# empymod/emg3d

Hardware: AMD Instinct MI355X
Metric: Mcells/s per multigrid cycle (higher is better)
Workload: dtype c128

## Files before the change

emg3d_amd/csrc/mg.hpp:

```cpp
#pragma once
#include <algorithm>
#include <cmath>
#include <cstdlib>
#include <cstring>
#include <map>
#include <memory>
#include <mutex>
#include <chrono>
#include <vector>

#include "common.hpp"
#include "smooth.hpp"
#include "stencil.hpp"
#include "smooth_qpl.hpp"
#include "smooth_qc.hpp"
#include "smooth_thm.hpp"
#include "smooth_tha.hpp"
#include "sweep_launch.hpp"
#include "sweep_plan.hpp"

template <class T>
struct Level {
    i64 nC[3];
    i64 nE, nCells;
// ... 869 lines not shown
        a.fac = L.fac[dir];
        a.fcomp = L.fac_kind[dir] == 4;
        if (L.fac_kind[dir] == 3) {
            a.mid = L.fac_mid[dir];
            const i64 nQ_ = L.nC[a.Q];
            const i64 nmax_ = a.nA[0] * ((nQ_ - 0) / 2);
            a.mode = 3;
            if (nmax_ > 0)
                MG_LAUNCH(k_line_factor_m<T>, dim3((unsigned)((nmax_ + EMG_LINE_BLOCK - 1) / EMG_LINE_BLOCK), 4),
                                   dim3(EMG_LINE_BLOCK), 0, stream, a);
            check_launch();
            return;
        }
        a.mid = L.fac_mid[dir];
        const i64 nQ = L.nC[a.Q];
        const i64 nB[2] = {(nQ - 0) / 2, (nQ - 1) / 2};
        a.mode = 3; a.cP = a.cQ = 0; a.cntA = a.cntB = 0;
        const i64 nmax = a.nA[0] * nB[0];
#ifdef EMG3D_LAB
        if (LAB_ENV("EMG3D_FACTOR_PER_COLOUR", 0)) {
            for (int c = 0; c < 4; ++c) {
                a.mode = 0; a.cP = c & 1; a.cQ = c >> 1; a.cntA = a.nA[a.cP]; a.cntB = nB[a.cQ];
                const i64 n = a.cntA * a.cntB;
                if (n > 0)
                    MG_LAUNCH(k_line_factor<T>, dim3((unsigned)((n + EMG_LINE_BLOCK - 1) / EMG_LINE_BLOCK)),
                                       dim3(EMG_LINE_BLOCK), 0, stream, a);
            }
            check_launch();
            return;
        }
#endif
        if (nmax > 0)
            MG_LAUNCH(k_line_factor<T>, dim3((unsigned)((nmax + EMG_LINE_BLOCK - 1) / EMG_LINE_BLOCK), 4),
                               dim3(EMG_LINE_BLOCK), 0, stream, a);
        check_launch();
    }

    unsigned xcd_grid(i64 nb) const { return (unsigned)(xcd_map ? ((nb + 7) / 8) * 8 : nb); }
    unsigned rp_grid(i64 nt) const { return xcd_grid((nt + EMG_RP_BLOCK - 1) / EMG_RP_BLOCK); }
    void ensure_qdesc(Level<T>& L, int dir) {
        const SweepPlan& P = plan(L, dir);
        if (!P.qdesc || L.qd[dir][0] || L.qdn[dir][0] == ~0u) return;
        L.qdn[dir][0] = ~0u;
        if (!L.fac[dir]) return;
        LineArgs<T> a;
        line_args(L, dir, a, true);
        const i64 lpg = 16 / a.seg;
        a.bt = Batch();
        for (int c = 0; c < 4; ++c) {
            a.mode = 0; a.cP = c & 1; a.cQ = c >> 1;
            a.cntA = a.nA[a.cP]; a.cntB = a.nB2[a.cQ];
            a.rs.slot0 = (unsigned)a.base[c];
            const i64 n = a.cntA * a.cntB;
            if (n <= 0) continue;
            const unsigned grid = xcd_grid((n + lpg - 1) / lpg);
            const i64 nthreads = (i64)grid * 64;
            void* tab = try_alloc<char>(nthreads * a.qM * (3 * 16 + 8 * 16));
            if (!tab) return;
            a.qd = tab; a.qdn = (unsigned)nthreads;
            if (!broken) qpl_launch<T>(1, a.qM, false, 1, false, dim3(grid), stream, a);
            L.qd[dir][c] = tab; L.qdn[dir][c] = (unsigned)nthreads;
        }
        check_launch();
    }
    char sweep_name[64] = "";
    char res_name[64] = "";
    int thm_lifo = (int)LAB_ENV("EMG3D_THM_LIFO", 0);
    void thm_attrs() {
#ifdef EMG3D_LAB
        static bool done[64] = {false};
        if (device < 0 || device >= 64 || done[device]) return;
        done[device] = true;
        thm_lifo_attrs<T>();
#endif
    }
    void launch_sweep(const SweepPlan& P, const LineArgs<T>& a, i64 n) {
        if (log_launches) fprintf(stderr, "[sweep] nC %lld %lld %lld L %d lines %lld kernel %s split %d\n", (long long)a.nC[0], (long long)a.nC[1], (long long)a.nC[2], a.L, (long long)n,
                                  P.name, a.split);
        memcpy(sweep_name, P.name, sizeof sweep_name);
        if (broken) return;
        switch (P.family) {
        case SweepFamily::tha: {
            const size_t dyn = P.helpers == 2 ? tha_lds_bytes<T, 2>((int)a.nC[a.L]) : tha_lds_bytes<T, 3>((int)a.nC[a.L]);
            tha_launch<T>(P.helpers, a.zsep != 0, bgrid(xcd_grid((n + THA_LPW - 1) / THA_LPW)), dyn, stream, a);
            break;
        }
        case SweepFamily::thm: {
            const i64 npairs = (n + P.inst_lpw - 1) / P.inst_lpw;
            thm_launch<T>(P.stages, P.inst_lpw, thm_lifo != 0, a.zsep != 0, bgrid(rp_grid(npairs * 128)), stream, a);
            break;
        }
        case SweepFamily::qpl:
        case SweepFamily::qpl_chain: {
            const i64 lpg = (16 * P.NW) / P.seg;
            qpl_launch<T>(P.NW, P.M, false, (P.NW == 1 && a.qd) ? 2 : 0, P.family == SweepFamily::qpl_chain,
                          bgrid(xcd_grid((n + lpg - 1) / lpg)), stream, a);
            break;
        }
        case SweepFamily::qc:
        case SweepFamily::qc_big: {
            LineArgs<T> b = a;
            b.qlpw = P.inst_lpw == 16 ? sweep_balanced_lpw(knobs, n * nsys) : P.inst_lpw;
            qc_launch<T>(P.stages, P.inst_lpw, a.zsep != 0, P.big, bgrid(rp_grid(((n + b.qlpw - 1) / b.qlpw) * 64)), stream, b);
            break;
        }
        case SweepFamily::rp: {
            const unsigned g = rp_grid(((n + P.inst_lpw - 1) / P.inst_lpw) * 64);
            if (P.inst_lpw == 8) hipLaunchKernelGGL((k_line_sweep_rp<T, 8>), bgrid(g), dim3(EMG_RP_BLOCK), 0, stream, a);
            else if (P.inst_lpw == 12) hipLaunchKernelGGL((k_line_sweep_rp<T, 12>), bgrid(g), dim3(EMG_RP_BLOCK), 0, stream, a);
            else hipLaunchKernelGGL((k_line_sweep_rp<T, 4>), bgrid(g), dim3(EMG_RP_BLOCK), 0, stream, a);
            break;
        }
        case SweepFamily::tpl:
            hipLaunchKernelGGL(k_line_sweep<T>, bgrid_y((unsigned)((n + EMG_LINE_BLOCK - 1) / EMG_LINE_BLOCK)), dim3(EMG_LINE_BLOCK), 0, stream, a);
            break;
        }
    }

    void prepare_work(Level<T>& L, int dir) {
        ensure_sflags(L, dir);
        if (home_on(L) || home_lvl(L)) ensure_work(L, 1);
        if (split_on(L)) ensure_work(L, (dir == 0) ? 0 : 1);
        else if (plan(L, dir).xt) ensure_transposed_model(L);
    }
    void to_work(Level<T>& L, int dir) {
        ensure_sflags(L, dir);
        if (split_on(L)) {
            const int w = (dir == 0) ? 0 : 1;
            ensure_work(L, w);
            if (home_lvl(L)) {
                if (w == 0) {
                    if (!L.sW_valid[0]) { convert_field(L, L.sW[0], L.sW[1], 2, true); L.sW_valid[0] = true; }
                    convert_field(L, L.eW[0], L.eW[1], 2, true);
                }
                return;
            }
            if (!L.sW_valid[w]) { convert_field(L, L.sW[w], L.s, w, true); L.sW_valid[w] = true; }
            if (!home_on(L)) convert_field(L, L.eW[w], L.e, w, true);
            else {
                e_to_w1(L);
                if (w == 0) convert_field(L, L.eW[0], L.eW[1], 2, true);
            }
        } else if (plan(L, dir).xt) {
            if (!L.sT_valid) { convert_field(L, L.sT, L.s, -1, true); L.sT_valid = true; }
            convert_field(L, L.eT, L.e, -1, true);
        }
    }
    void from_work(Level<T>& L, int dir) {
        if (home_on(L) || home_lvl(L)) {
            if (dir == 0) convert_field(L, L.eW[1], L.eW[0], 2, false);
        } else if (split_on(L)) convert_field(L, L.e, L.eW[(dir == 0) ? 0 : 1], (dir == 0) ? 0 : 1, false);
        else if (plan(L, dir).xt) convert_field(L, L.e, L.eT, -1, false);
    }
    int work_id(Level<T>& L, int dir) { return plan(L, dir).work_id; }

    int place_tries = getenv("EMG3D_PLACE_TRIES") ? atoi(getenv("EMG3D_PLACE_TRIES")) : 12;
    i64 place_min_bytes = LAB_ENV("EMG3D_PLACE_MIN_MB", 256) << 20;
    int place_reps = (int)LAB_ENV("EMG3D_PLACE_REPS", 1);
    double place_gap = 1.075;
    static const int PLACE_MAX = 16;
    struct PlaceRec { int tries = 0, kept = 0, reused = 0; float ms[PLACE_MAX] = {0}; };
    PlaceRec place_rec[2];
    bool placed[2] = {false, false};
    static bool lr_has(int lr, int dir) {
        return dir == 0 ? (lr == 1 || lr == 5 || lr == 6 || lr == 7) : dir == 1 ? (lr == 2 || lr == 4 || lr == 6 || lr == 7)
                                                                              : (lr == 3 || lr == 4 || lr == 5 || lr == 7);
    }
// ... 419 lines not shown
```

emg3d_amd/csrc/smooth_tha.hpp:

```cpp
#pragma once
#include "smooth_thm.hpp"

struct ThaPair { double a, b; };

constexpr int THA_LPW = 8;
constexpr int THA_MAX_DYN_LDS = 140 * 1024;
constexpr int THA_STATIC_LDS = 18 * 1024;
template <int NH> constexpr int tha_ring_depth() { return 8; }
template <class T, int NH>
inline size_t tha_lds_bytes(int nL) {
    const size_t KS = (size_t)((nL + 1) / 2);
    return ((size_t)2 * tha_ring_depth<NH>() * 5 + (size_t)2 * (KS + 2)) * (5 * THA_LPW) * sizeof(T);
}

template <int NH> constexpr int tha_threads() { return 64 * (2 + 2 * NH); }
template <class T, int NH, bool ZS = false>
__global__ __launch_bounds__(tha_threads<NH>()) void k_line_sweep_tha(LineArgs<T> a) {
    typedef unsigned int u32;
    constexpr int LPW = THA_LPW, D = tha_ring_depth<NH>(), NW = tha_threads<NH>() / 64, L40 = 5 * LPW;
    const int lane = threadIdx.x & 63;
    const int wave = __builtin_amdgcn_readfirstlane(threadIdx.x >> 6);
    const int H = wave & 1;
    const int hj = (wave >> 1) - 1;
    const int q = lane / LPW;
    const int g = lane - q * LPW;
    thm_args_burst(a);
    __shared__ int prod[2][4];
    __shared__ int cons[2];
    __shared__ int mid[2];
    if (threadIdx.x < 8) (&prod[0][0])[threadIdx.x] = 0;
    if (threadIdx.x >= 8 && threadIdx.x < 10) cons[threadIdx.x - 8] = 0;
    if (threadIdx.x >= 10 && threadIdx.x < 12) mid[threadIdx.x - 10] = 0;
    __syncthreads();
#ifdef EMG3D_LAB
    const bool ts_on = (a.tile & 256) && blockIdx.x == 0 && lane == 0 && H == 0;
    long long ts[6] = {0, 0, 0, 0, 0, 0};
    __shared__ long long ts0;
#define THA_TS(i) do { if (ts_on) ts[i] = (long long)__builtin_readcyclecounter(); } while (0)
    if (ts_on && hj < 0) ts0 = (long long)__builtin_readcyclecounter();
#else
#define THA_TS(i) do {} while (0)
#endif
    THA_TS(0);
    EMG_SWEEP_WG(a)
    const u32 gidx = (u32)wg * LPW + g;
    const u32 cA = (u32)a.cntA;
    if (gidx >= cA * (u32)a.cntB) return;
    const u32 bq = gidx / cA, qq = gidx - bq * cA;
    const u32 jP = 1u + (u32)a.cP + 2u * qq, jQ = 1u + (u32)a.cQ + 2u * bq;
    const int n = (int)a.rs.nL;
    const int m = (int)a.mid;
    const int K = H ? n - m - 2 : m;
    const int KS = (n + 1) / 2;
    const u32 slot = a.rs.slot0 + gidx;
    const u32 nLt = (u32)a.nLinesTot;
    const u32 csL = a.rs.csL, csP = a.rs.csP, csQ = a.rs.csQ;
    const double ihP[2] = {a.rs.ihP[jP - 1], a.rs.ihP[jP]};
    const double ihQ[2] = {a.rs.ihQ[jQ - 1], a.rs.ihQ[jQ]};
    const double kP[2] = {0.5 * ihP[0], 0.5 * ihP[1]};
    const double kQ[2] = {0.5 * ihQ[0], 0.5 * ihQ[1]};
    const u32 jPm = jP - 1, jPp = jP + 1, jQm = jQ - 1, jQp = jQ + 1;
    const bool spl = (a.split & 1) != 0;
    const u32 nPc = a.rs.nP, nPn = a.rs.nP + 1u;
    const u32 spsh = spl ? 1u : 0u, sphc = spl ? (nPc + 1u) >> 1 : 0u, sphn = spl ? (nPn + 1u) >> 1 : 0u;
    auto spc = [&](u32 v) -> u32 { return (v >> spsh) + (v & spsh) * sphc; };
    auto spn = [&](u32 v) -> u32 { return (v >> spsh) + (v & spsh) * sphn; };
#define FL_(vL, vP, vQ) (a.rs.off[0] + (vL) * a.rs.st[0][0] + spn(vP) * a.rs.st[0][1] + (vQ) * a.rs.st[0][2])
#define FP_(vL, vP, vQ) (a.rs.off[1] + (vL) * a.rs.st[1][0] + spc(vP) * a.rs.st[1][1] + (vQ) * a.rs.st[1][2])
#define FQ_(vL, vP, vQ) (a.rs.off[2] + (vL) * a.rs.st[2][0] + spn(vP) * a.rs.st[2][1] + (vQ) * a.rs.st[2][2])
    const u32 cP0 = spc(jP - 1) * csP, cP1 = spc(jP) * csP, cq = (jQ - 1) * csQ;

    const bool rowact = q < 5;
    const int rr = rowact ? q : 0;
    const int type = (rr == 0) ? 0 : (rr <= 2 ? 1 : 2);
    const int side = (rr == 0) ? 0 : ((rr - 1) & 1);
    const double sg = side ? -1.0 : 1.0;
    const double tmask = (type == 0) ? 0.0 : 1.0;
    u32 ob[7], os[7];
    u32 fb, sv, suT0;
    double Kc[6];
    double ca = 0.0;
    if (type == 0) {
        ob[0] = FL_(0, jP, jQ);
        ob[1] = FL_(0, jPp, jQ); ob[2] = FL_(0, jPm, jQ); ob[3] = FL_(0, jP, jQp); ob[4] = FL_(0, jP, jQm);
        ob[5] = ob[1]; ob[6] = ob[1];
#pragma unroll
        for (int t = 0; t < 7; ++t) os[t] = a.rs.st[0][0];
        fb = cP0 + cq; sv = csQ; suT0 = cP1 - cP0;
        Kc[0] = kP[1] * ihP[1]; Kc[1] = kP[0] * ihP[0]; Kc[2] = kQ[1] * ihQ[1]; Kc[3] = kQ[0] * ihQ[0];
        Kc[4] = 0.0; Kc[5] = 0.0;
    } else if (type == 1) {
        const u32 pcell = jPm + side, pnode = side ? jPp : jPm;
        ob[0] = FP_(1, pcell, jQ);
        ob[1] = FL_(1, pnode, jQ); ob[2] = FL_(0, pnode, jQ);
        ob[3] = FQ_(1, pnode, jQ); ob[4] = FQ_(1, pnode, jQm);
        ob[5] = FP_(1, pcell, jQp); ob[6] = FP_(1, pcell, jQm);
        os[0] = a.rs.st[1][0]; os[1] = a.rs.st[0][0]; os[2] = a.rs.st[0][0];
        os[3] = a.rs.st[2][0]; os[4] = a.rs.st[2][0]; os[5] = a.rs.st[1][0]; os[6] = a.rs.st[1][0];
        fb = (side ? cP1 : cP0) + cq; sv = csQ; suT0 = 0;
        const double ihA = ihP[side];
        Kc[0] = sg * ihA; Kc[1] = -sg * ihA;
        Kc[2] = sg * kQ[1] * ihA; Kc[3] = -sg * kQ[0] * ihA;
        Kc[4] = kQ[1] * ihQ[1]; Kc[5] = kQ[0] * ihQ[0];
        ca = sg * 0.5 * ihA;
    } else {
        const u32 qcell = jQm + side, qnode = side ? jQp : jQm;
        ob[0] = FQ_(1, jP, qcell);
        ob[1] = FL_(1, jP, qnode); ob[2] = FL_(0, jP, qnode);
// ... 44 lines not shown
    const u32 wst = 15u * nLt * TS;
    u32 eo[6], es[6];
#pragma unroll
    for (int t = 0; t < 6; ++t) { eo[t] = ob[1 + t] * TS; es[t] = os[1 + t] * TS; }
    const u32 so = ob[0] * TS, ss = os[0] * TS;
    const u32 zo0 = fb * 8u, zo1 = (fb + sv) * 8u;
    const u32 zsu = suT0 * 8u, zsL = csL * 8u;

    extern __shared__ __attribute__((aligned(16))) char tha_dyn_lds[];
    const int l40 = rr * LPW + g;
    T* const ring = reinterpret_cast<T*>(tha_dyn_lds) + (size_t)H * (D * 5 * L40) + l40;
    T* const zs = reinterpret_cast<T*>(tha_dyn_lds) + (size_t)2 * (D * 5 * L40) + (size_t)H * ((KS + 2) * L40);
    __shared__ T xy_[NW][64];
    __shared__ ThaPair xc_[NW][64];
    __shared__ T jn[2][6 * LPW];
    T* const xy = xy_[wave];
    ThaPair* const xc = xc_[wave];

    auto own_idx = [&](int ic) -> u32 {
        int v = t0 ? ic : (H ? ic - 1 : ic);
        const int hi = t0 ? n - 1 : n - 2;
        v = v < 0 ? 0 : (v > hi ? hi : v);
        return (u32)v;
    };
    auto fwd_block = [&](int k) -> int { return H ? n - 1 - k : k; };
    auto bwd_block = [&](int k) -> int { return H ? m + 2 + k : m - 1 - k; };
    auto rhs = [&](const TmStep<T>& cur, double& czb, double& cza, double& kLb, double& kLa) -> T {
        kLb = 0.5 * cur.ihl0; kLa = 0.5 * cur.ihl1;
        const double f0 = ZS ? zeta_of(0, cur.zf[0]) : cur.zf[0], f1 = ZS ? zeta_of(1, cur.zf[0]) : cur.zf[1];
        const double f2 = ZS ? zeta_of(2, cur.zf[2]) : cur.zf[2], f3 = ZS ? zeta_of(3, cur.zf[2]) : cur.zf[3];
        const double rs0 = f0 + f1, rs1 = f2 + f3;
        const double cs0 = f0 + f2, cs1 = f1 + f3;
        const double g0 = (t0 ? Kc[0] : Kc[0] * kLa) * rs1;
        const double g1 = (t0 ? Kc[1] : Kc[1] * kLb) * rs0;
        T y = cur.S;
        y += g0 * cur.E[0];
        y += g1 * cur.E[1];
        y += (Kc[2] * cs1) * cur.E[2];
        y += (Kc[3] * cs0) * cur.E[3];
        y += (Kc[4] * cs1) * cur.E[4];
        y += (Kc[5] * cs0) * cur.E[5];
        czb = rs0 * cur.ihl0;
        cza = rs1 * cur.ihl1;
        return y;
    };
    auto load_rhs = [&](u32 ix, TmStep<T>& d) {
        const u32 su = t0 ? zsu : zsL;
        const u32 zb = __umul24(ix, zsL);
        if (ZS) {
            d.zf[0] = *reinterpret_cast<const double*>(wLB + ix * 8u);
            d.zf[2] = *reinterpret_cast<const double*>(wLB + (t0 ? ix : ix + 1u) * 8u);
        } else {
            d.zf[0] = *reinterpret_cast<const double*>(zB + (zb + zo0));
            d.zf[1] = *reinterpret_cast<const double*>(zB + (zb + zo1));
            d.zf[2] = *reinterpret_cast<const double*>(zB + (zb + zo0 + su));
            d.zf[3] = *reinterpret_cast<const double*>(zB + (zb + zo1 + su));
        }
        d.ihl0 = *reinterpret_cast<const double*>(hB + ix * 8u);
        d.ihl1 = *reinterpret_cast<const double*>(hB + (t0 ? ix : ix + 1u) * 8u);
        d.S = nosrc ? Zero<T>::v() : *reinterpret_cast<const T*>(sB + (so + __umul24(ix, ss)));
#pragma unroll
        for (int t = 0; t < 6; ++t) d.E[t] = *reinterpret_cast<const T*>(eB + (eo[t] + __umul24(ix, es[t])));
    };
#ifdef EMG3D_LAB
    long long ts_wait = 0;
#endif
    auto wait_ge = [&](int* p, int v, int& seen) {
        if (seen >= v) return;
#ifdef EMG3D_LAB
        const long long w0 = ts_on ? (long long)__builtin_readcyclecounter() : 0;
#endif
        while ((seen = __hip_atomic_load(p, __ATOMIC_ACQUIRE, __HIP_MEMORY_SCOPE_WORKGROUP)) < v) __builtin_amdgcn_s_sleep(1);
#ifdef EMG3D_LAB
        if (ts_on) ts_wait += (long long)__builtin_readcyclecounter() - w0;
#endif
    };

    if (hj >= 0) {
        if (!rowact) return;
        int cons_seen = 0;
        auto publish = [&](int gs) {
            if (lane == 0) __hip_atomic_store(&prod[H][hj], gs + 1, __ATOMIC_RELEASE, __HIP_MEMORY_SCOPE_WORKGROUP);
        };
        auto load_f = [&](int k_, TmStep<T>& d) {
            const int ic_ = fwd_block(k_ < K ? k_ : K - 1);
            load_rhs(own_idx(ic_), d);
            const u32 wb = __umul24((u32)ic_, wst);
#pragma unroll
            for (int c = 0; c < 5; ++c) d.W[c] = *reinterpret_cast<const T*>(wB + (wb + wo[c]));
        };
        auto produce_f = [&](const TmStep<T>& cur, int k_) {
            double czb, cza, kLb, kLa;
            const T y = rhs(cur, czb, cza, kLb, kLa);
            const double cz = H ? cza : czb;
            const double kk = H ? kLa : kLb;
            ThaPair cc; cc.a = (tmask * kk) * cz; cc.b = cah * cz;
            xy[lane] = y;
            xc[lane] = cc;
            const T Y0 = xy[g], Y1 = xy[g + LPW], Y2 = xy[g + 2 * LPW], Y3 = xy[g + 3 * LPW], Y4 = xy[g + 4 * LPW];
            const ThaPair C1 = xc[g + LPW], C2 = xc[g + 2 * LPW], C3 = xc[g + 3 * LPW], C4 = xc[g + 4 * LPW];
            const T av = ((cur.W[0] * Y0 + cur.W[1] * Y1) + (cur.W[2] * Y2 + cur.W[3] * Y3)) + cur.W[4] * Y4;
            const T G1 = cur.W[1] * C1.a - cur.W[0] * C1.b, G2 = cur.W[2] * C2.a - cur.W[0] * C2.b;
            const T G3 = cur.W[3] * C3.a - cur.W[0] * C3.b, G4 = cur.W[4] * C4.a - cur.W[0] * C4.b;
            wait_ge(&cons[H], k_ - D + 1, cons_seen);
            if (rowact) {
                T* const s_ = ring + (size_t)((u32)k_ % (u32)D) * (5 * L40);
                s_[0] = av; s_[L40] = G1; s_[2 * L40] = G2; s_[3 * L40] = G3; s_[4 * L40] = G4;
            }
            publish(k_);
        };
        THA_TS(1);
        {
            TmStep<T> bA, bB;
            int k = hj;
            if (k < K) load_f(k, bA);
            for (; k < K; k += 2 * NH) {
                if (k + NH < K) load_f(k + NH, bB);
                produce_f(bA, k);
                if (k + NH < K) {
                    if (k + 2 * NH < K) load_f(k + 2 * NH, bA);
                    produce_f(bB, k + NH);
                }
            }
        }
        THA_TS(2);
        struct BwdIn { T W[5]; double p0, p1, ihc; };
        auto load_b = [&](int kb_, BwdIn& d) {
            const int ic_ = bwd_block(kb_);
            const u32 wb = __umul24((u32)ic_, wst);
#pragma unroll
            for (int c = 1; c < 5; ++c) d.W[c] = *reinterpret_cast<const T*>(wB + (wb + wo[c]));
            const int ci = H ? ic_ - 1 : ic_ + 1;
            const u32 zb = __umul24((u32)ci, zsL);
            if (ZS) {
                d.p0 = *reinterpret_cast<const double*>(wLB + (u32)ci * 8u);
            } else {
                d.p0 = *reinterpret_cast<const double*>(zB + (zb + zo0));
                d.p1 = *reinterpret_cast<const double*>(zB + (zb + zo1));
            }
            d.ihc = *reinterpret_cast<const double*>(hB + (u32)ci * 8u);
        };
        auto produce_b = [&](const BwdIn& bc, int kb_) {
            const double cz = (ZS ? zeta_of(0, bc.p0) + zeta_of(1, bc.p0) : bc.p0 + bc.p1) * bc.ihc;
            ThaPair cc; cc.a = cah * cz; cc.b = ((-0.5 * tmask) * bc.ihc) * cz;
            xc[lane] = cc;
            const ThaPair C1 = xc[g + LPW], C2 = xc[g + 2 * LPW], C3 = xc[g + 3 * LPW], C4 = xc[g + 4 * LPW];
            const T h0 = (bc.W[1] * C1.a + bc.W[2] * C2.a) + (bc.W[3] * C3.a + bc.W[4] * C4.a);
            const int gs = K + kb_;
            wait_ge(&cons[H], gs - D + 1, cons_seen);
            if (rowact) {
                T* const s_ = ring + (size_t)((u32)gs % (u32)D) * (5 * L40);
                s_[0] = -h0; s_[L40] = -(bc.W[1] * C1.b); s_[2 * L40] = -(bc.W[2] * C2.b);
                s_[3 * L40] = -(bc.W[3] * C3.b); s_[4 * L40] = -(bc.W[4] * C4.b);
            }
            publish(gs);
        };
        {
            BwdIn bA, bB;
            int k = hj;
            if (k < K) load_b(k, bA);
            for (; k < K; k += 2 * NH) {
                if (k + NH < K) load_b(k + NH, bB);
                produce_b(bA, k);
                if (k + NH < K) {
                    if (k + 2 * NH < K) load_b(k + 2 * NH, bA);
                    produce_b(bB, k + NH);
                }
            }
        }
        THA_TS(3);
#ifdef EMG3D_LAB
        if (ts_on) printf("[tha helper %d] entry %lld setup %lld fwd done %lld bwd done %lld (cycles after the chain wave's entry), waiting for ring space %lld\n",
                          hj, ts[0] - ts0, ts[1] - ts0, ts[2] - ts0, ts[3] - ts0, ts_wait);
#endif
        return;
    }

    const int icm = H ? m + 1 : m;
    TmStep<T> cur;
    load_rhs((u32)(t0 ? icm : m), cur);
    const int ur = H ? 5 : rr;
    T Wm[6];
#pragma unroll
    for (int c = 0; c < 6; ++c) {
        const int r1 = ur > c ? ur : c, c1 = ur > c ? c : ur;
        const int p = r1 * (r1 + 1) / 2 + c1;
        const u32 blk = p < 15 ? (u32)m : (u32)m + 1u;
        const int ent = p < 15 ? p : p - 15;
        Wm[c] = *reinterpret_cast<const T*>(wB + (__umul24(blk, wst) + ((u32)ent * nLt + slot) * TS));
    }
    int prod_seen[NH];
#pragma unroll
    for (int j = 0; j < NH; ++j) prod_seen[j] = 0;
    auto consumed = [&](int gs) {
        asm volatile("" ::: "memory");
        if (lane == 0) __hip_atomic_store(&cons[H], gs + 1, __ATOMIC_RELAXED, __HIP_MEMORY_SCOPE_WORKGROUP);
    };
    THA_TS(1);
    T* const zrow = zs + l40;
    const T* const zcol = zs + g;
    zrow[0] = Zero<T>::v();
    T zprev = Zero<T>::v();
    auto fwd_step = [&](int k_, int j_) {
        wait_ge(&prod[H][j_], k_ + 1, prod_seen[j_]);
        const T* const s_ = ring + (size_t)((u32)k_ % (u32)D) * (5 * L40);
        const T av = s_[0], G1 = s_[L40], G2 = s_[2 * L40], G3 = s_[3 * L40], G4 = s_[4 * L40];
        const T* const zc = zcol + (size_t)k_ * L40;
        const T Z1 = zc[LPW], Z2 = zc[2 * LPW], Z3 = zc[3 * LPW], Z4 = zc[4 * LPW];
        T z = av;
        T z2 = G2 * Z2;
        cmac(z, G1, Z1);
        cmac(z2, G4, Z4);
        cmac(z, G3, Z3);
        z = z + z2;
        zrow[(size_t)(k_ + 1) * L40] = z;
        zprev = z;
        consumed(k_);
    };
    {
        int k = 0;
        for (; k + NH <= K; k += NH) {
#pragma unroll
            for (int j = 0; j < NH; ++j) fwd_step(k + j, j);
        }
#pragma unroll
        for (int j = 0; j < NH; ++j) if (k + j < K) fwd_step(k + j, j);
    }
    THA_TS(2);
#ifdef EMG3D_LAB
    ts[5] = ts_wait;
#endif
    auto pair_sync = [&](int epoch) {
        if (lane == 0) __hip_atomic_store(&mid[H], epoch, __ATOMIC_RELEASE, __HIP_MEMORY_SCOPE_WORKGROUP);
        while (__hip_atomic_load(&mid[1 - H], __ATOMIC_ACQUIRE, __HIP_MEMORY_SCOPE_WORKGROUP) < epoch) __builtin_amdgcn_s_sleep(1);
    };
    pair_sync(1);
    {
        double czb, cza, kLb, kLa;
        T y = rhs(cur, czb, cza, kLb, kLa);
        const T zL = H ? Zero<T>::v() : zprev;
        const int KR = n - m - 2;
        const T zR = (reinterpret_cast<T*>(tha_dyn_lds) + (size_t)2 * (D * 5 * L40) + (size_t)((KS + 2) * L40))[(size_t)KR * L40 + l40];
        if (!H) {
            y += ((tmask * kLb) * czb) * zL;
            y += ((tmask * kLa) * cza) * zR;
            xy[lane] = (ca * czb) * zL;
        } else {
            xy[lane] = (ca * cza) * zR;
        }
        const T su = (xy[g + LPW] + xy[g + 2 * LPW]) + (xy[g + 3 * LPW] + xy[g + 4 * LPW]);
        if (t0) y = H ? y + su : y - su;
        if (rowact) {
            if (!H) jn[0][rr * LPW + g] = y;
            else if (t0) jn[0][5 * LPW + g] = y;
        }
        pair_sync(2);
        T x = Zero<T>::v();
#pragma unroll
        for (int c = 0; c < 6; ++c) x += Wm[c] * jn[0][c * LPW + g];
        if (rowact && (!H || t0)) jn[1][(H ? 5 : rr) * LPW + g] = x;
        pair_sync(3);
        if (rowact && (!H || t0)) {
            if (!H) *reinterpret_cast<T*>(eWr + (so + __umul24((u32)m, ss))) = x;
            else *reinterpret_cast<T*>(eWr + (so + __umul24((u32)(m + 1), ss))) = x;
        }
        zprev = jn[1][(t0 ? (H ? 5 : 0) : rr) * LPW + g];
        zrow[(size_t)(K + 1) * L40] = zprev;
    }
    THA_TS(3);
    u32 xo = so + __umul24(own_idx(bwd_block(0)), ss);
    const u32 dxo = H ? ss : 0u - ss;
    auto bwd_step = [&](int kb_, int j_) {
        const int gs = K + kb_;
        wait_ge(&prod[H][j_], gs + 1, prod_seen[j_]);
        const T* const s_ = ring + (size_t)((u32)gs % (u32)D) * (5 * L40);
        const T H0 = s_[0], H1 = s_[L40], H2 = s_[2 * L40], H3 = s_[3 * L40], H4 = s_[4 * L40];
        const int kz = K - kb_;
        const T zi = zrow[(size_t)kz * L40];
        const T* const xc_in = zcol + (size_t)(kz + 1) * L40;
        const T X0 = xc_in[0], X1 = xc_in[LPW], X2 = xc_in[2 * LPW], X3 = xc_in[3 * LPW], X4 = xc_in[4 * LPW];
        T x = zi;
        T x2 = H1 * X1;
        cmac(x, H0, X0);
        cmac(x2, H3, X3);
        cmac(x, H2, X2);
        cmac(x2, H4, X4);
        x = x + x2;
        zrow[(size_t)kz * L40] = x;
        *reinterpret_cast<T*>(eWr + xo) = x;
        xo += dxo;
        consumed(gs);
    };
    {
        int k = 0;
        for (; k + NH <= K; k += NH) {
#pragma unroll
            for (int j = 0; j < NH; ++j) bwd_step(k + j, j);
        }
#pragma unroll
        for (int j = 0; j < NH; ++j) if (k + j < K) bwd_step(k + j, j);
    }
    THA_TS(4);
#ifdef EMG3D_LAB
    if (ts_on) printf("[tha chain L] K %d: setup %lld forward %lld middle %lld backward %lld (cycles after entry), waiting for helpers %lld (%lld of it in the forward steps)\n", K,
                      ts[1] - ts[0], ts[2] - ts[0], ts[3] - ts[0], ts[4] - ts[0], ts_wait, ts[5]);
#endif
#undef THA_TS
}
```

emg3d_amd/csrc/sweep_launch.hpp:

```cpp
#pragma once
#include "smooth.hpp"
#include "stencil.hpp"

template <class T> void qc_launch(int stages, int lpw, bool zsep, bool big, dim3 grid, hipStream_t st, const LineArgs<T>& a);

template <class T> void thm_launch(int stages, int lpw, bool lifo, bool zsep, dim3 grid, hipStream_t st, const LineArgs<T>& a);
template <class T> void thm_lifo_attrs();

template <class T> void tha_launch(int helpers, bool zsep, dim3 grid, size_t dyn_lds, hipStream_t st, const LineArgs<T>& a);
template <class T> bool tha_attrs(int max_dyn_lds);

template <class T> void qpl_launch(int nw, int m, bool hl, int dm, bool chain, dim3 grid, hipStream_t st, const LineArgs<T>& a);

template <class T> void residual_launch(int mode, int kz, dim3 grid, hipStream_t st, const ResidualArgs<T>& a);
```

emg3d_amd/csrc/sweep_plan.hpp:

```cpp
#pragma once
#include <algorithm>
#include <cstdint>
#include <cstdio>
#include <cstdlib>

typedef int64_t i64;

#ifndef LAB_ENV
#ifdef EMG3D_LAB
inline long long lab_env_(const char* name, long long def) { const char* v = getenv(name); return v ? atoll(v) : def; }
inline int lab_env_ch_(const char* name) { const char* v = getenv(name); return v ? v[0] : 0; }
#define LAB_ENV(name, def) lab_env_(name, (long long)(def))
#define LAB_ENV_CH(name) lab_env_ch_(name)
#else
#define LAB_ENV(name, def) ((long long)(def))
#define LAB_ENV_CH(name) 0
#endif
#endif

constexpr int SWEEP_THA_LPW = 8, SWEEP_THA_RING = 8, SWEEP_THA_MAX_DYN_LDS = 140 * 1024, SWEEP_THA_STATIC_LDS = 18 * 1024;
inline i64 sweep_tha_lds_bytes(i64 nL, int tsize) {
    return (2 * SWEEP_THA_RING * 5 + 2 * ((nL + 1) / 2 + 2)) * (5 * SWEEP_THA_LPW) * (i64)tsize;
}

struct SweepKnobs {
    i64 simds = 1024;
    i64 lds_limit = 160 * 1024;
    bool tha_lds_granted = true;
    int order = 1, nsys = 1;
    int batch_tune = getenv("EMG3D_BATCH_TUNE") ? atoi(getenv("EMG3D_BATCH_TUNE")) : 0;

    int sweep_kernel = LAB_ENV_CH("EMG3D_SWEEP") == 't' ? 1 : 0;
    bool use_xt = LAB_ENV("EMG3D_XT", 1) != 0;
    i64 xt_min_cells = LAB_ENV("EMG3D_XT_MIN", 8192);
    int th_lpw = (int)LAB_ENV("EMG3D_TH_LPW", 0);
    int force_lpw = (int)LAB_ENV("EMG3D_LPW", 0);
    bool use_twist = LAB_ENV("EMG3D_TWIST", 1) != 0;
    i64 twist_max_lines_env = LAB_ENV("EMG3D_TWIST_MAX", 0);
    int tw_stages = (int)LAB_ENV("EMG3D_TW_STAGES", 0);
    int use_split = (int)LAB_ENV("EMG3D_SPLIT", 2);
    i64 split_min_cells = LAB_ENV("EMG3D_SPLIT_MIN_CELLS", 2000000);
    int use_q = (int)LAB_ENV("EMG3D_Q", 1);
    i64 q_min_lines_env = LAB_ENV("EMG3D_Q_MIN_LINES", 0);
    int q_stages = (int)LAB_ENV("EMG3D_Q_STAGES", 0);
    int q_lpw = (int)LAB_ENV("EMG3D_Q_LPW", 0);
    int q_big_lab = (int)LAB_ENV("EMG3D_Q_BIG", 0);
    int use_qpl = (int)LAB_ENV("EMG3D_QPL", 7);
    i64 qpl_min_nl = LAB_ENV("EMG3D_QPL_MIN", 2);
    i64 qpl_max_nl = LAB_ENV("EMG3D_QPL_MAX_NL", 64);
    i64 qpl_m2_min = LAB_ENV("EMG3D_QPL_M2", 32);
    int qpl_chain_seg = (int)LAB_ENV("EMG3D_QPL_CHAIN", 4);
    i64 qpl_few_lines_env = LAB_ENV("EMG3D_QPL_FEW", 0);
    i64 qpl_max_lines = LAB_ENV("EMG3D_QPL_MAX", (i64)1 << 40);
    int use_qdesc = (int)LAB_ENV("EMG3D_QDESC", 1);
    i64 qdesc_max_threads_env = LAB_ENV("EMG3D_QDESC_MAX", 0);
    int use_tha = (int)LAB_ENV("EMG3D_THA", 3);
    i64 tha_min_nl = LAB_ENV("EMG3D_THA_MIN", 33), tha_mid_nl = LAB_ENV("EMG3D_THA_MID", 64), tha_min_lines_env = LAB_ENV("EMG3D_THA_MIN_LINES", 0);
    i64 tha_max_nl = LAB_ENV("EMG3D_THA_MAX", 128);
    i64 tha_big_max_lines_env = LAB_ENV("EMG3D_THA_BIG_LINES", 0);
    int tha_split = (int)LAB_ENV("EMG3D_THA_SPLIT", 0);

    i64 q_min_lines() const { return q_min_lines_env > 0 ? q_min_lines_env : 8 * simds; }
    i64 twist_max_lines() const { return twist_max_lines_env > 0 ? twist_max_lines_env : q_min_lines(); }
    i64 qpl_few_lines() const { return qpl_few_lines_env > 0 ? qpl_few_lines_env : simds; }
    i64 qdesc_max_threads() const { return qdesc_max_threads_env > 0 ? qdesc_max_threads_env : (9000 * simds + 1023) / 1024; }
    i64 tha_min_lines() const { return tha_min_lines_env > 0 ? tha_min_lines_env : (1100 * simds + 1023) / 1024; }
    i64 tha_big_max_lines() const { return tha_big_max_lines_env > 0 ? tha_big_max_lines_env : (i64)SWEEP_THA_LPW * (simds / 4); }
};

struct SweepShape {
    i64 nC[3];
    int tsize;
    i64 cells() const { return nC[0] * nC[1] * nC[2]; }
    i64 edges() const {
        return nC[0] * (nC[1] + 1) * (nC[2] + 1) + (nC[0] + 1) * nC[1] * (nC[2] + 1) + (nC[0] + 1) * (nC[1] + 1) * nC[2];
    }
    i64 lines(int dir) const { return (nC[dir == 0 ? 1 : 0] / 2) * (nC[dir == 2 ? 1 : 2] / 2); }
    i64 lines_tot(int dir) const { return (nC[dir == 0 ? 1 : 0] - 1) * (nC[dir == 2 ? 1 : 2] - 1); }
    i64 field_stride(int c, int ax, bool transposed) const {
        const i64 d0 = (c == 0) ? nC[0] : nC[0] + 1, d1 = (c == 1) ? nC[1] : nC[1] + 1;
        return ax == 2 ? d0 * d1 : ((ax == 0) != transposed) ? 1 : (transposed ? d1 : d0);
    }
    i64 cell_stride(int ax, bool transposed) const {
        return ax == 2 ? nC[0] * nC[1] : ((ax == 0) != transposed) ? 1 : (transposed ? nC[1] : nC[0]);
    }
};

enum class SweepFamily { tpl, rp, qc, qc_big, thm, tha, qpl, qpl_chain };

inline void sweep_kernel_name(char* out, size_t len, SweepFamily f, int tsize, int p1 = 0, int p2 = 0) {
    static const char* const base[] = {"k_line_sweep", "k_line_sweep_rp", "k_line_sweep_qc", "k_line_sweep_qc_big", "k_line_sweep_thm",
                                       "k_line_sweep_tha", "k_line_sweep_qpl", "k_line_sweep_qpl_chain"};
    const char* tn = tsize == 16 ? "c128" : "f64";
    if (f == SweepFamily::tpl) snprintf(out, len, "%s<%s>", base[(int)f], tn);
    else if (f == SweepFamily::rp || f == SweepFamily::tha) snprintf(out, len, "%s<%s,%d>", base[(int)f], tn, p1);
    else snprintf(out, len, "%s<%s,%d,%d>", base[(int)f], tn, p1, p2);
}

struct SweepPlan {
    SweepFamily family = SweepFamily::tpl;
    int stages = 0, inst_lpw = 0, helpers = 0, NW = 0, M = 0, seg = 0;
    int qlpw = 0;
    bool big = false;
    bool split = false;
    bool xt = false;
    int work_id = 0;
    int fac_kind = 0;
    i64 fac_entries = 0;
    i64 mid = 0;
    bool qdesc = false;
    i64 nmax = 0;
    i64 lpw = 0;
    i64 rounds = 0;
    char name[64] = "";
};

inline bool sweep_wide_fits(const SweepKnobs& K, const SweepShape& G) {
    const i64 lim = (i64)1 << 32;
    const i64 mx = std::max(G.lines_tot(0), std::max(G.lines_tot(1), G.lines_tot(2)));
    return K.sweep_kernel == 0 && mx * 15 * (i64)G.tsize < lim && G.cells() * 8 < lim;
}
inline bool sweep_q_big_lines(const SweepKnobs& K, const SweepShape& G) {
    for (int d = 0; d < 3; ++d) if (G.lines(d) < std::max<i64>(K.q_min_lines(), 1)) return false;
    return K.order == 1 && K.use_q >= 1;
}
inline bool sweep_q_big(const SweepKnobs& K, const SweepShape& G) {
    return sweep_wide_fits(K, G) && sweep_q_big_lines(K, G) && (K.q_big_lab || G.edges() * (i64)G.tsize >= ((i64)1 << 32));
}
inline bool sweep_rp_fits(const SweepKnobs& K, const SweepShape& G) {
    return sweep_wide_fits(K, G) && G.edges() * (i64)G.tsize < ((i64)1 << 32) && !(K.q_big_lab && sweep_q_big_lines(K, G));
}
inline bool sweep_split_on(const SweepKnobs& K, const SweepShape& G) {
    return (K.use_split == 1 || (K.use_split == 2 && K.order == 1 && G.cells() >= K.split_min_cells)) &&
           (sweep_rp_fits(K, G) || sweep_q_big(K, G));
}

inline int sweep_tha_helpers(const SweepKnobs& K, const SweepShape& G, int dir) {
    if ((K.use_tha != 3 && K.use_tha != 2) || K.order != 1 || K.sweep_kernel != 0 || !K.use_twist || !sweep_rp_fits(K, G)) return 0;
    const i64 nL = G.nC[dir], lds = sweep_tha_lds_bytes(nL, G.tsize);
    if (nL < K.tha_min_nl || nL > K.tha_max_nl) return 0;
    if (!K.tha_lds_granted || lds > SWEEP_THA_MAX_DYN_LDS || lds + SWEEP_THA_STATIC_LDS > K.lds_limit) return 0;
    const bool big = nL > K.tha_mid_nl;
    if (!big && sweep_split_on(K, G) && !K.tha_split) return 0;
    const i64 lines = G.lines(dir);
    if (lines < K.tha_min_lines() || lines >= K.q_min_lines()) return 0;
    if (big && lines > K.tha_big_max_lines()) return 0;
    return K.use_tha;
}
inline bool sweep_qpl_on(const SweepKnobs& K, const SweepShape& G, int dir) {
    if (!((K.use_qpl >> dir) & 1) || sweep_split_on(K, G) || K.sweep_kernel != 0 || sweep_tha_helpers(K, G, dir)) return false;
    const i64 nL = G.nC[dir], cap = (nL >= K.qpl_m2_min) ? 256 : 128;
    i64 lines = G.lines(dir), max_nl = K.qpl_max_nl;
    if (K.batch_tune && K.nsys > 1 && K.order == 1) {
        lines *= K.nsys;
        max_nl = std::max<i64>(4, K.qpl_max_nl / K.nsys);
    }
    const i64 maxnl = (K.order == 0 || lines <= K.qpl_few_lines()) ? cap : std::min<i64>(max_nl, cap);
    if (nL < K.qpl_min_nl || nL > maxnl || !sweep_rp_fits(K, G)) return false;
    return lines <= K.qpl_max_lines;
}
inline bool sweep_twist_ok(const SweepKnobs& K, const SweepShape& G, int dir, bool q_on, bool transposed) {
    if (q_on || !K.use_twist || !sweep_rp_fits(K, G) || G.nC[dir] < 3) return false;
    if (G.lines(dir) >= K.twist_max_lines()) return false;
    const i64 lim24 = (i64)1 << 24;
    i64 mxs = 15 * G.lines_tot(dir) * (i64)G.tsize;
    for (int c = 0; c < 3; ++c) mxs = std::max(mxs, G.field_stride(c, dir, transposed) * (i64)G.tsize);
    mxs = std::max(mxs, G.cell_stride(dir, transposed) * 8);
    const i64 fac_bytes = 15 * G.lines_tot(dir) * G.nC[dir] * (i64)G.tsize;
    return mxs < lim24 && G.nC[dir] < lim24 && fac_bytes < ((i64)1 << 32);
}
inline int sweep_balanced_lpw(const SweepKnobs& K, i64 lines) {
    const i64 rounds = std::max<i64>(1, (lines + 16 * K.simds - 1) / (16 * K.simds));
    const i64 lpw = (lines + K.simds * rounds - 1) / (K.simds * rounds);
    return (int)std::min<i64>(16, std::max<i64>(lpw, 8));
}

inline SweepPlan plan_sweep(const SweepKnobs& K, const SweepShape& G, int dir) {
    SweepPlan p;
    const i64 nL = G.nC[dir], nmax = G.lines(dir), S = K.simds;
    const bool rp_fits = sweep_rp_fits(K, G), qpl = sweep_qpl_on(K, G, dir);
    p.nmax = nmax;
    p.split = sweep_split_on(K, G);
    p.xt = dir == 0 && K.use_xt && G.cells() >= K.xt_min_cells && !qpl;
    p.work_id = p.split ? (dir == 0 ? 0 : 1) : (p.xt ? 2 : 3 + dir);
    p.big = sweep_q_big(K, G) && !rp_fits;
    p.helpers = sweep_tha_helpers(K, G, dir);
    const bool q_on = K.use_q >= 2 || (K.use_q == 1 && nmax >= K.q_min_lines());
    p.fac_kind = (!qpl && sweep_twist_ok(K, G, dir, q_on, p.xt)) ? 3 : (!qpl && (rp_fits || p.big) && q_on) ? 4 : 0;
    p.mid = p.fac_kind == 3 ? (nL - 1) / 2 : nL - 1;
    p.fac_entries = (p.fac_kind == 4 ? 11 : 15) * nL;
    int p1 = 0, p2 = 0;
    if (p.fac_kind == 3 && p.helpers) {
        p.family = SweepFamily::tha;
        p1 = p.helpers;
        p.lpw = SWEEP_THA_LPW; p.rounds = (((nmax + p.lpw - 1) / p.lpw) * K.nsys + S / 4 - 1) / (S / 4);
    } else if (p.fac_kind == 3) {
        p.family = SweepFamily::thm;
        const i64 lines = nmax * K.nsys, r8 = (2 * ((lines + 7) / 8) + S - 1) / S, r12 = (2 * ((lines + 11) / 12) + S - 1) / S;
        p.inst_lpw = (K.th_lpw == 4 || K.th_lpw == 8 || K.th_lpw == 12) ? K.th_lpw : (23 * r12 < 20 * r8) ? 12 : 8;
        p.stages = K.tw_stages ? K.tw_stages : 3;
        p1 = p.stages; p2 = p.inst_lpw;
        p.lpw = p.inst_lpw; p.rounds = (2 * ((nmax + p.lpw - 1) / p.lpw) * K.nsys + S - 1) / S;
    } else if (qpl) {
        p.M = (nL >= K.qpl_m2_min) ? 2 : 1;
        p.seg = 4; while (p.seg < (nL + p.M - 1) / p.M) p.seg *= 2;
        p.NW = p.seg <= 16 ? 1 : p.seg / 16;
        p.family = (p.NW == 1 && p.M == 1 && K.order == 1 && p.seg <= K.qpl_chain_seg) ? SweepFamily::qpl_chain : SweepFamily::qpl;
        p1 = p.NW; p2 = p.M;
        p.fac_entries = 15 * (i64)p.M * p.seg;
        p.lpw = (16 * p.NW) / p.seg; p.rounds = (((nmax + p.lpw - 1) / p.lpw) * p.NW * K.nsys + S - 1) / S;
        p.qdesc = K.use_qdesc && K.order == 1 && p.NW == 1 && G.lines_tot(dir) * p.fac_entries < ((i64)1 << 32) &&
                  ((nmax + p.lpw - 1) / p.lpw) * 64 <= K.qdesc_max_threads();
    } else if ((rp_fits || p.big) && p.fac_kind == 4) {
        p.family = p.big ? SweepFamily::qc_big : SweepFamily::qc;
        p.inst_lpw = p.big ? 16 : K.q_lpw ? K.q_lpw : (nmax >= K.q_min_lines() ? 16 : 4);
        p.stages = (K.q_stages == 2 || K.q_stages == 3) ? K.q_stages
                 : (p.inst_lpw == 16 && nmax * K.nsys > 15 * S && nmax * K.nsys <= 16 * S) ? 2 : 3;
        p.qlpw = p.inst_lpw == 16 ? sweep_balanced_lpw(K, nmax * K.nsys) : p.inst_lpw;
        p1 = p.stages; p2 = p.inst_lpw;
        p.lpw = p.qlpw; p.rounds = (((nmax + p.lpw - 1) / p.lpw) * K.nsys + S - 1) / S;
    } else if (rp_fits || p.big) {
        p.family = SweepFamily::rp;
        p.lpw = K.force_lpw ? K.force_lpw : (nmax >= 8 * S ? 8 : 4);
        p.inst_lpw = (p.lpw == 8 || p.lpw == 12) ? (int)p.lpw : 4;
        p1 = p.inst_lpw;
        p.rounds = (((nmax + p.lpw - 1) / p.lpw) * K.nsys + S - 1) / S;
    } else {
        p.family = SweepFamily::tpl;
        p.lpw = 64; p.rounds = (((nmax + 63) / 64) * K.nsys + S - 1) / S;
    }
    sweep_kernel_name(p.name, sizeof p.name, p.family, G.tsize, p1, p2);
    return p;
}
```

emg3d_amd/csrc/sweep_tha.hip:

```cpp
#include "sweep_launch.hpp"
#ifndef EMG3D_UNIT_T
#define EMG3D_UNIT_T 2
#endif
#include "smooth_tha.hpp"

template <class T, int NH>
static void tha_launch_h(bool zsep, dim3 grid, size_t dyn, hipStream_t st, const LineArgs<T>& a) {
    if (zsep) hipLaunchKernelGGL((k_line_sweep_tha<T, NH, true>), grid, dim3(tha_threads<NH>()), dyn, st, a);
    else hipLaunchKernelGGL((k_line_sweep_tha<T, NH, false>), grid, dim3(tha_threads<NH>()), dyn, st, a);
}
template <class T>
void tha_launch(int helpers, bool zsep, dim3 grid, size_t dyn_lds, hipStream_t st, const LineArgs<T>& a) {
#ifdef EMG3D_LAB
    if (helpers == 2) { tha_launch_h<T, 2>(zsep, grid, dyn_lds, st, a); return; }
#endif
    (void)helpers;
    tha_launch_h<T, 3>(zsep, grid, dyn_lds, st, a);
}
#if EMG3D_UNIT_T != 1
template void tha_launch<double>(int, bool, dim3, size_t, hipStream_t, const LineArgs<double>&);
#endif
#if EMG3D_UNIT_T != 0
template void tha_launch<c128>(int, bool, dim3, size_t, hipStream_t, const LineArgs<c128>&);
#endif

template <class T>
bool tha_attrs(int max_dyn_lds) {
    bool ok = true;
    auto dyn_lds = [&](const void* f) {
        if (hipFuncSetAttribute(f, hipFuncAttributeMaxDynamicSharedMemorySize, max_dyn_lds) != hipSuccess) { (void)hipGetLastError(); ok = false; }
    };
    dyn_lds(reinterpret_cast<const void*>(&k_line_sweep_tha<T, 3, false>));
    dyn_lds(reinterpret_cast<const void*>(&k_line_sweep_tha<T, 3, true>));
#ifdef EMG3D_LAB
    dyn_lds(reinterpret_cast<const void*>(&k_line_sweep_tha<T, 2, false>));
    dyn_lds(reinterpret_cast<const void*>(&k_line_sweep_tha<T, 2, true>));
#endif
    return ok;
}
#if EMG3D_UNIT_T != 1
template bool tha_attrs<double>(int);
#endif
#if EMG3D_UNIT_T != 0
template bool tha_attrs<c128>(int);
#endif
```

Before: 249.0.

## Pack three THA helper waves onto four-step rounds with 12-lane groups

Adds a packed helper mapping for the three-helper THA line-sweep kernel. Each helper wave now covers 12 lanes per group instead of 8, so the three helpers together produce four ring steps per round rather than three. The consumer waits on two producers for the shared step. The packed variant becomes the default launched kernel. The aim is better lane utilisation in the producer waves, at the cost of more complex synchronisation and some lanes with uneven work.

```diff
diff --git a/emg3d_amd/csrc/mg.hpp b/emg3d_amd/csrc/mg.hpp
--- a/emg3d_amd/csrc/mg.hpp
+++ b/emg3d_amd/csrc/mg.hpp
@@ -975,7 +975,7 @@
         switch (P.family) {
         case SweepFamily::tha: {
             const size_t dyn = P.helpers == 2 ? tha_lds_bytes<T, 2>((int)a.nC[a.L]) : tha_lds_bytes<T, 3>((int)a.nC[a.L]);
-            tha_launch<T>(P.helpers, a.zsep != 0, bgrid(xcd_grid((n + THA_LPW - 1) / THA_LPW)), dyn, stream, a);
+            tha_launch<T>(P.helpers, P.pack, a.zsep != 0, bgrid(xcd_grid((n + THA_LPW - 1) / THA_LPW)), dyn, stream, a);
             break;
         }
         case SweepFamily::thm: {
diff --git a/emg3d_amd/csrc/smooth_tha.hpp b/emg3d_amd/csrc/smooth_tha.hpp
--- a/emg3d_amd/csrc/smooth_tha.hpp
+++ b/emg3d_amd/csrc/smooth_tha.hpp
@@ -14,16 +14,28 @@
 }
 
 template <int NH> constexpr int tha_threads() { return 64 * (2 + 2 * NH); }
-template <class T, int NH, bool ZS = false>
+constexpr int THA_RND = 4;
+template <class T, int NH, bool ZS = false, bool PK = false>
 __global__ __launch_bounds__(tha_threads<NH>()) void k_line_sweep_tha(LineArgs<T> a) {
+    static_assert(!PK || (NH == 3 && tha_ring_depth<NH>() >= 2 * THA_RND), "the packed helper map is written for three helpers and a ring of two rounds");
     typedef unsigned int u32;
     constexpr int LPW = THA_LPW, D = tha_ring_depth<NH>(), NW = tha_threads<NH>() / 64, L40 = 5 * LPW;
     const int lane = threadIdx.x & 63;
     const int wave = __builtin_amdgcn_readfirstlane(threadIdx.x >> 6);
     const int H = wave & 1;
     const int hj = (wave >> 1) - 1;
-    const int q = lane / LPW;
-    const int g = lane - q * LPW;
+    int q = lane / LPW;
+    int g = lane - q * LPW;
+    int xu = g, ds = 0, dlo = 0, dhi = 0;
+    constexpr int XS = PK ? 12 : LPW;
+    if (PK && hj >= 0) {
+        q = lane / 12;
+        xu = lane - q * 12;
+        g = xu < 8 ? xu : (hj == 1 ? xu - 8 : xu - 4);
+        ds = hj == 0 ? 0 : hj == 1 ? (xu < 8 ? 1 : 2) : (xu < 8 ? 3 : 2);
+        dlo = hj == 2 ? 2 : hj; dhi = hj == 0 ? 0 : hj + 1;
+        if (hj == 0 && xu >= 8) q = 5;
+    }
     thm_args_burst(a);
     __shared__ int prod[2][4];
     __shared__ int cons[2];
@@ -234,6 +246,9 @@
         auto publish = [&](int gs) {
             if (lane == 0) __hip_atomic_store(&prod[H][hj], gs + 1, __ATOMIC_RELEASE, __HIP_MEMORY_SCOPE_WORKGROUP);
         };
+        const int kst = PK ? ds : hj;
+        constexpr int KSTEP = PK ? THA_RND : NH;
+        auto khi_of = [&](int k0_) -> int { const int v = k0_ + dhi; return v < K ? v : K - 1; };
         auto load_f = [&](int k_, TmStep<T>& d) {
             const int ic_ = fwd_block(k_ < K ? k_ : K - 1);
             load_rhs(own_idx(ic_), d);
@@ -241,7 +256,7 @@
 #pragma unroll
             for (int c = 0; c < 5; ++c) d.W[c] = *reinterpret_cast<const T*>(wB + (wb + wo[c]));
         };
-        auto produce_f = [&](const TmStep<T>& cur, int k_) {
+        auto produce_f = [&](const TmStep<T>& cur, int k_, int khi) {
             double czb, cza, kLb, kLa;
             const T y = rhs(cur, czb, cza, kLb, kLa);
             const double cz = H ? cza : czb;
@@ -249,36 +264,37 @@
             ThaPair cc; cc.a = (tmask * kk) * cz; cc.b = cah * cz;
             xy[lane] = y;
             xc[lane] = cc;
-            const T Y0 = xy[g], Y1 = xy[g + LPW], Y2 = xy[g + 2 * LPW], Y3 = xy[g + 3 * LPW], Y4 = xy[g + 4 * LPW];
-            const ThaPair C1 = xc[g + LPW], C2 = xc[g + 2 * LPW], C3 = xc[g + 3 * LPW], C4 = xc[g + 4 * LPW];
+            const T Y0 = xy[xu], Y1 = xy[xu + XS], Y2 = xy[xu + 2 * XS], Y3 = xy[xu + 3 * XS], Y4 = xy[xu + 4 * XS];
+            const ThaPair C1 = xc[xu + XS], C2 = xc[xu + 2 * XS], C3 = xc[xu + 3 * XS], C4 = xc[xu + 4 * XS];
             const T av = ((cur.W[0] * Y0 + cur.W[1] * Y1) + (cur.W[2] * Y2 + cur.W[3] * Y3)) + cur.W[4] * Y4;
             const T G1 = cur.W[1] * C1.a - cur.W[0] * C1.b, G2 = cur.W[2] * C2.a - cur.W[0] * C2.b;
             const T G3 = cur.W[3] * C3.a - cur.W[0] * C3.b, G4 = cur.W[4] * C4.a - cur.W[0] * C4.b;
-            wait_ge(&cons[H], k_ - D + 1, cons_seen);
-            if (rowact) {
+            wait_ge(&cons[H], khi - D + 1, cons_seen);
+            if (rowact && (!PK || k_ < K)) {
                 T* const s_ = ring + (size_t)((u32)k_ % (u32)D) * (5 * L40);
                 s_[0] = av; s_[L40] = G1; s_[2 * L40] = G2; s_[3 * L40] = G3; s_[4 * L40] = G4;
             }
-            publish(k_);
+            publish(khi);
         };
         THA_TS(1);
         {
             TmStep<T> bA, bB;
-            int k = hj;
-            if (k < K) load_f(k, bA);
-            for (; k < K; k += 2 * NH) {
-                if (k + NH < K) load_f(k + NH, bB);
-                produce_f(bA, k);
-                if (k + NH < K) {
-                    if (k + 2 * NH < K) load_f(k + 2 * NH, bA);
-                    produce_f(bB, k + NH);
+            const int klo = PK ? dlo : hj, ko = kst - klo;
+            int k = klo;
+            if (k < K) load_f(k + ko, bA);
+            for (; k < K; k += 2 * KSTEP) {
+                if (k + KSTEP < K) load_f(k + KSTEP + ko, bB);
+                produce_f(bA, k + ko, PK ? khi_of(k - klo) : k);
+                if (k + KSTEP < K) {
+                    if (k + 2 * KSTEP < K) load_f(k + 2 * KSTEP + ko, bA);
+                    produce_f(bB, k + KSTEP + ko, PK ? khi_of(k + KSTEP - klo) : k + KSTEP);
                 }
             }
         }
         THA_TS(2);
         struct BwdIn { T W[5]; double p0, p1, ihc; };
         auto load_b = [&](int kb_, BwdIn& d) {
-            const int ic_ = bwd_block(kb_);
+            const int ic_ = bwd_block(PK ? (kb_ < K ? kb_ : K - 1) : kb_);
             const u32 wb = __umul24((u32)ic_, wst);
 #pragma unroll
             for (int c = 1; c < 5; ++c) d.W[c] = *reinterpret_cast<const T*>(wB + (wb + wo[c]));
@@ -292,31 +308,32 @@
             }
             d.ihc = *reinterpret_cast<const double*>(hB + (u32)ci * 8u);
         };
-        auto produce_b = [&](const BwdIn& bc, int kb_) {
+        auto produce_b = [&](const BwdIn& bc, int kb_, int khi) {
             const double cz = (ZS ? zeta_of(0, bc.p0) + zeta_of(1, bc.p0) : bc.p0 + bc.p1) * bc.ihc;
             ThaPair cc; cc.a = cah * cz; cc.b = ((-0.5 * tmask) * bc.ihc) * cz;
             xc[lane] = cc;
-            const ThaPair C1 = xc[g + LPW], C2 = xc[g + 2 * LPW], C3 = xc[g + 3 * LPW], C4 = xc[g + 4 * LPW];
+            const ThaPair C1 = xc[xu + XS], C2 = xc[xu + 2 * XS], C3 = xc[xu + 3 * XS], C4 = xc[xu + 4 * XS];
             const T h0 = (bc.W[1] * C1.a + bc.W[2] * C2.a) + (bc.W[3] * C3.a + bc.W[4] * C4.a);
             const int gs = K + kb_;
-            wait_ge(&cons[H], gs - D + 1, cons_seen);
-            if (rowact) {
+            wait_ge(&cons[H], K + khi - D + 1, cons_seen);
+            if (rowact && (!PK || kb_ < K)) {
                 T* const s_ = ring + (size_t)((u32)gs % (u32)D) * (5 * L40);
                 s_[0] = -h0; s_[L40] = -(bc.W[1] * C1.b); s_[2 * L40] = -(bc.W[2] * C2.b);
                 s_[3 * L40] = -(bc.W[3] * C3.b); s_[4 * L40] = -(bc.W[4] * C4.b);
             }
-            publish(gs);
+            publish(K + khi);
         };
         {
             BwdIn bA, bB;
-            int k = hj;
-            if (k < K) load_b(k, bA);
-            for (; k < K; k += 2 * NH) {
-                if (k + NH < K) load_b(k + NH, bB);
-                produce_b(bA, k);
-                if (k + NH < K) {
-                    if (k + 2 * NH < K) load_b(k + 2 * NH, bA);
-                    produce_b(bB, k + NH);
+            const int klo = PK ? dlo : hj, ko = kst - klo;
+            int k = klo;
+            if (k < K) load_b(k + ko, bA);
+            for (; k < K; k += 2 * KSTEP) {
+                if (k + KSTEP < K) load_b(k + KSTEP + ko, bB);
+                produce_b(bA, k + ko, PK ? khi_of(k - klo) : k);
+                if (k + KSTEP < K) {
+                    if (k + 2 * KSTEP < K) load_b(k + 2 * KSTEP + ko, bA);
+                    produce_b(bB, k + KSTEP + ko, PK ? khi_of(k + KSTEP - klo) : k + KSTEP);
                 }
             }
         }
@@ -353,8 +370,9 @@
     const T* const zcol = zs + g;
     zrow[0] = Zero<T>::v();
     T zprev = Zero<T>::v();
-    auto fwd_step = [&](int k_, int j_) {
+    auto fwd_step = [&](int k_, int j_, int j2_ = -1) {
         wait_ge(&prod[H][j_], k_ + 1, prod_seen[j_]);
+        if (j2_ >= 0) wait_ge(&prod[H][j2_], k_ + 1, prod_seen[j2_]);
         const T* const s_ = ring + (size_t)((u32)k_ % (u32)D) * (5 * L40);
         const T av = s_[0], G1 = s_[L40], G2 = s_[2 * L40], G3 = s_[3 * L40], G4 = s_[4 * L40];
         const T* const zc = zcol + (size_t)k_ * L40;
@@ -369,7 +387,13 @@
         zprev = z;
         consumed(k_);
     };
-    {
+    if constexpr (PK) {
+        int k = 0;
+        for (; k + THA_RND <= K; k += THA_RND) { fwd_step(k, 0); fwd_step(k + 1, 1); fwd_step(k + 2, 1, 2); fwd_step(k + 3, 2); }
+        if (k < K) fwd_step(k, 0);
+        if (k + 1 < K) fwd_step(k + 1, 1);
+        if (k + 2 < K) fwd_step(k + 2, 1, 2);
+    } else {
         int k = 0;
         for (; k + NH <= K; k += NH) {
 #pragma unroll
@@ -422,9 +446,10 @@
     THA_TS(3);
     u32 xo = so + __umul24(own_idx(bwd_block(0)), ss);
     const u32 dxo = H ? ss : 0u - ss;
-    auto bwd_step = [&](int kb_, int j_) {
+    auto bwd_step = [&](int kb_, int j_, int j2_ = -1) {
         const int gs = K + kb_;
         wait_ge(&prod[H][j_], gs + 1, prod_seen[j_]);
+        if (j2_ >= 0) wait_ge(&prod[H][j2_], gs + 1, prod_seen[j2_]);
         const T* const s_ = ring + (size_t)((u32)gs % (u32)D) * (5 * L40);
         const T H0 = s_[0], H1 = s_[L40], H2 = s_[2 * L40], H3 = s_[3 * L40], H4 = s_[4 * L40];
         const int kz = K - kb_;
@@ -443,7 +468,13 @@
         xo += dxo;
         consumed(gs);
     };
-    {
+    if constexpr (PK) {
+        int k = 0;
+        for (; k + THA_RND <= K; k += THA_RND) { bwd_step(k, 0); bwd_step(k + 1, 1); bwd_step(k + 2, 1, 2); bwd_step(k + 3, 2); }
+        if (k < K) bwd_step(k, 0);
+        if (k + 1 < K) bwd_step(k + 1, 1);
+        if (k + 2 < K) bwd_step(k + 2, 1, 2);
+    } else {
         int k = 0;
         for (; k + NH <= K; k += NH) {
 #pragma unroll
diff --git a/emg3d_amd/csrc/sweep_launch.hpp b/emg3d_amd/csrc/sweep_launch.hpp
--- a/emg3d_amd/csrc/sweep_launch.hpp
+++ b/emg3d_amd/csrc/sweep_launch.hpp
@@ -7,7 +7,7 @@
 template <class T> void thm_launch(int stages, int lpw, bool lifo, bool zsep, dim3 grid, hipStream_t st, const LineArgs<T>& a);
 template <class T> void thm_lifo_attrs();
 
-template <class T> void tha_launch(int helpers, bool zsep, dim3 grid, size_t dyn_lds, hipStream_t st, const LineArgs<T>& a);
+template <class T> void tha_launch(int helpers, bool pack, bool zsep, dim3 grid, size_t dyn_lds, hipStream_t st, const LineArgs<T>& a);
 template <class T> bool tha_attrs(int max_dyn_lds);
 
 template <class T> void qpl_launch(int nw, int m, bool hl, int dm, bool chain, dim3 grid, hipStream_t st, const LineArgs<T>& a);
diff --git a/emg3d_amd/csrc/sweep_plan.hpp b/emg3d_amd/csrc/sweep_plan.hpp
--- a/emg3d_amd/csrc/sweep_plan.hpp
+++ b/emg3d_amd/csrc/sweep_plan.hpp
@@ -58,6 +58,7 @@
     i64 tha_min_nl = LAB_ENV("EMG3D_THA_MIN", 33), tha_mid_nl = LAB_ENV("EMG3D_THA_MID", 64), tha_min_lines_env = LAB_ENV("EMG3D_THA_MIN_LINES", 0);
     i64 tha_max_nl = LAB_ENV("EMG3D_THA_MAX", 128);
     i64 tha_big_max_lines_env = LAB_ENV("EMG3D_THA_BIG_LINES", 0);
+    int tha_pack = (int)LAB_ENV("EMG3D_THA_PACK", 1);
     int tha_split = (int)LAB_ENV("EMG3D_THA_SPLIT", 0);
 
     i64 q_min_lines() const { return q_min_lines_env > 0 ? q_min_lines_env : 8 * simds; }
@@ -100,6 +101,7 @@
 struct SweepPlan {
     SweepFamily family = SweepFamily::tpl;
     int stages = 0, inst_lpw = 0, helpers = 0, NW = 0, M = 0, seg = 0;
+    bool pack = false;
     int qlpw = 0;
     bool big = false;
     bool split = false;
@@ -185,6 +187,7 @@
     p.work_id = p.split ? (dir == 0 ? 0 : 1) : (p.xt ? 2 : 3 + dir);
     p.big = sweep_q_big(K, G) && !rp_fits;
     p.helpers = sweep_tha_helpers(K, G, dir);
+    p.pack = p.helpers == 3 && K.tha_pack != 0;
     const bool q_on = K.use_q >= 2 || (K.use_q == 1 && nmax >= K.q_min_lines());
     p.fac_kind = (!qpl && sweep_twist_ok(K, G, dir, q_on, p.xt)) ? 3 : (!qpl && (rp_fits || p.big) && q_on) ? 4 : 0;
     p.mid = p.fac_kind == 3 ? (nL - 1) / 2 : nL - 1;
diff --git a/emg3d_amd/csrc/sweep_tha.hip b/emg3d_amd/csrc/sweep_tha.hip
--- a/emg3d_amd/csrc/sweep_tha.hip
+++ b/emg3d_amd/csrc/sweep_tha.hip
@@ -4,24 +4,25 @@
 #endif
 #include "smooth_tha.hpp"
 
-template <class T, int NH>
+template <class T, int NH, bool PK>
 static void tha_launch_h(bool zsep, dim3 grid, size_t dyn, hipStream_t st, const LineArgs<T>& a) {
-    if (zsep) hipLaunchKernelGGL((k_line_sweep_tha<T, NH, true>), grid, dim3(tha_threads<NH>()), dyn, st, a);
-    else hipLaunchKernelGGL((k_line_sweep_tha<T, NH, false>), grid, dim3(tha_threads<NH>()), dyn, st, a);
+    if (zsep) hipLaunchKernelGGL((k_line_sweep_tha<T, NH, true, PK>), grid, dim3(tha_threads<NH>()), dyn, st, a);
+    else hipLaunchKernelGGL((k_line_sweep_tha<T, NH, false, PK>), grid, dim3(tha_threads<NH>()), dyn, st, a);
 }
 template <class T>
-void tha_launch(int helpers, bool zsep, dim3 grid, size_t dyn_lds, hipStream_t st, const LineArgs<T>& a) {
+void tha_launch(int helpers, bool pack, bool zsep, dim3 grid, size_t dyn_lds, hipStream_t st, const LineArgs<T>& a) {
 #ifdef EMG3D_LAB
-    if (helpers == 2) { tha_launch_h<T, 2>(zsep, grid, dyn_lds, st, a); return; }
+    if (helpers == 2) { tha_launch_h<T, 2, false>(zsep, grid, dyn_lds, st, a); return; }
+    if (!pack) { tha_launch_h<T, 3, false>(zsep, grid, dyn_lds, st, a); return; }
 #endif
-    (void)helpers;
-    tha_launch_h<T, 3>(zsep, grid, dyn_lds, st, a);
+    (void)helpers; (void)pack;
+    tha_launch_h<T, 3, true>(zsep, grid, dyn_lds, st, a);
 }
 #if EMG3D_UNIT_T != 1
-template void tha_launch<double>(int, bool, dim3, size_t, hipStream_t, const LineArgs<double>&);
+template void tha_launch<double>(int, bool, bool, dim3, size_t, hipStream_t, const LineArgs<double>&);
 #endif
 #if EMG3D_UNIT_T != 0
-template void tha_launch<c128>(int, bool, dim3, size_t, hipStream_t, const LineArgs<c128>&);
+template void tha_launch<c128>(int, bool, bool, dim3, size_t, hipStream_t, const LineArgs<c128>&);
 #endif
 
 template <class T>
@@ -30,9 +31,11 @@
     auto dyn_lds = [&](const void* f) {
         if (hipFuncSetAttribute(f, hipFuncAttributeMaxDynamicSharedMemorySize, max_dyn_lds) != hipSuccess) { (void)hipGetLastError(); ok = false; }
     };
+    dyn_lds(reinterpret_cast<const void*>(&k_line_sweep_tha<T, 3, false, true>));
+    dyn_lds(reinterpret_cast<const void*>(&k_line_sweep_tha<T, 3, true, true>));
+#ifdef EMG3D_LAB
     dyn_lds(reinterpret_cast<const void*>(&k_line_sweep_tha<T, 3, false>));
     dyn_lds(reinterpret_cast<const void*>(&k_line_sweep_tha<T, 3, true>));
-#ifdef EMG3D_LAB
     dyn_lds(reinterpret_cast<const void*>(&k_line_sweep_tha<T, 2, false>));
     dyn_lds(reinterpret_cast<const void*>(&k_line_sweep_tha<T, 2, true>));
 #endif
```

Measured after the change: 248.2. No clear change (-0.4%).
